# duj12/ASR-2Pass

Hardware: AMD Instinct MI355X
Metric: audio-sec/sec (xRT) Paraformer-large offline, 30s utts (higher is better)
Workload: dtype f32 (operands staged as 2 fp16 planes = 22-23 significant bits, 3 products per block on the FP16 matrix cores, fp32 accumulate; error vs fp64 = the fp32 MFMA chain's)

## Files before the change

asr-2pass_amd/csrc/attention_x3.hip:

```cpp
#include "kernels.h"
#include "launch_common.h"
#include "split_common.h"

#include <math.h>

namespace pfhip {
namespace {

using f32x16 = __attribute__((ext_vector_type(16))) float;

#ifndef PFHIP_ATT_ABLATE
#define PFHIP_ATT_ABLATE 0
#endif
constexpr bool kAbNoFsmn = PFHIP_ATT_ABLATE == 1, kAbNoBar = PFHIP_ATT_ABLATE == 2 || PFHIP_ATT_ABLATE == 6,
               kAbNoSoftmax = PFHIP_ATT_ABLATE == 3 || PFHIP_ATT_ABLATE == 6, kAbOneV = PFHIP_ATT_ABLATE == 4 || PFHIP_ATT_ABLATE == 6,
               kAbNoStage = PFHIP_ATT_ABLATE == 5 || PFHIP_ATT_ABLATE == 6;
constexpr int kHD = 128, kQW = 32, kNW = 8, kQB = kNW * kQW, kKT = 32;
constexpr int kKRow = 272;
constexpr int kKPlane = kKT * kKRow;
constexpr int kVRow = 72;
constexpr int kVPlane = kHD * kVRow;
constexpr int kBuf = 2 * kKPlane + 2 * kVPlane;
constexpr int kOS = kHD + 4;
constexpr int kLdsBytes = kNW * kQW * kOS * 4;
static_assert(kLdsBytes >= 2 * kBuf, "K/V buffers must fit");


__global__ __launch_bounds__(512, 1) void attention_x3_kernel(
    const float* __restrict__ Q, int ldq, const float* __restrict__ K, int ldk, const float* __restrict__ V, int ldv,
    float* __restrict__ O, int ldo, const int* __restrict__ q_off, const int* __restrict__ q_len,
    const int* __restrict__ kv_off, const int* __restrict__ kv_len, float scale, const float* __restrict__ fsmn_w,
    float* mem, int ldmem, int mem_accumulate, unsigned char* __restrict__ Ph, unsigned char* __restrict__ Pl, int rows_p) {
  extern __shared__ __attribute__((aligned(16))) unsigned char lds[];

  const int b = blockIdx.y, head = blockIdx.x;
  const int Lq = q_len[b];
  const int q0 = blockIdx.z * kQB;
  if (q0 >= Lq) return;
  const int Lk = kv_len[b];
  const size_t qbase = (size_t)q_off[b], kbase = (size_t)kv_off[b];
  const int tid = threadIdx.x, lane = tid & 63, wave = tid >> 6;
  const int r = lane & 31, h = lane >> 5;

  if (fsmn_w && !kAbNoFsmn) {
    constexpr int kTaps = 11, kStrip = 16;
    const int cg = tid & 31, strip = tid >> 5;
    const int c = head * kHD + 4 * cg, t0 = q0 + strip * kStrip;
    if (t0 < Lk) {
      float wk[4][kTaps];
#pragma unroll
      for (int ch = 0; ch < 4; ++ch)
#pragma unroll
        for (int j = 0; j < kTaps; ++j) wk[ch][j] = fsmn_w[(size_t)(c + ch) * kTaps + j];
      float4 rows[kStrip + kTaps - 1];
#pragma unroll
      for (int j = 0; j < kStrip + kTaps - 1; ++j) {
        const int t = t0 - 5 + j;
        rows[j] = (t < 0 || t >= Lk) ? make_float4(0.f, 0.f, 0.f, 0.f) : *reinterpret_cast<const float4*>(V + (kbase + t) * ldv + c);
      }
#pragma unroll
      for (int s0 = 0; s0 < kStrip; s0 += 8) {
        float4 xo[8];
#pragma unroll
        for (int s = 0; s < 8; ++s) {
          const int t = t0 + s0 + s;
          xo[s] = (mem_accumulate && t < Lk) ? *reinterpret_cast<const float4*>(mem + (kbase + t) * ldmem + c)
                                             : make_float4(0.f, 0.f, 0.f, 0.f);
        }
#pragma unroll
        for (int s1 = 0; s1 < 8; ++s1) {
          const int s = s0 + s1, t = t0 + s;
          if (t < Lk) {
            float4 o = rows[s + 5];
            float4 a = make_float4(0.f, 0.f, 0.f, 0.f);
#pragma unroll
            for (int j = 0; j < kTaps; ++j) {
              a.x += wk[0][j] * rows[s + j].x;
              a.y += wk[1][j] * rows[s + j].y;
              a.z += wk[2][j] * rows[s + j].z;
              a.w += wk[3][j] * rows[s + j].w;
            }
            o.x += a.x; o.y += a.y; o.z += a.z; o.w += a.w;
            if (mem_accumulate) { o.x += xo[s1].x; o.y += xo[s1].y; o.z += xo[s1].z; o.w += xo[s1].w; }
            *reinterpret_cast<float4*>(mem + (kbase + t) * ldmem + c) = o;
          }
        }
      }
    }
  }

  half8 qf[8][2];
  {
    int qrow = q0 + wave * kQW + r;
    if (qrow >= Lq) qrow = Lq - 1;
    const float* qp = Q + (qbase + qrow) * ldq + head * kHD + 8 * h;
    const float qs = scale * 1.44269504088896340736f;
#pragma unroll
    for (int s = 0; s < 8; ++s) {
      const float4 a = *reinterpret_cast<const float4*>(qp + 16 * s);
      const float4 c = *reinterpret_cast<const float4*>(qp + 16 * s + 4);
      const float v[8] = {a.x * qs, a.y * qs, a.z * qs, a.w * qs, c.x * qs, c.y * qs, c.z * qs, c.w * qs};
      split8(v, qf[s][0], qf[s][1]);
    }
  }

  const int kkey = tid >> 4, kc = tid & 15;
  const float* Kh = K + kbase * ldk + head * kHD + 4 * kc;
  const int vd2 = tid & 63, vkg = tid >> 6;
  const float* Vh = V + kbase * ldv + head * kHD + 2 * vd2;
  float4 rk0, rk1;
  float2 rv0, rv1, rv2, rv3;
  auto load_tile = [&](int kt) {
    int key = kt * kKT + kkey;
    key = key < Lk ? key : Lk - 1;
    const float* kp = Kh + (size_t)key * ldk;
    rk0 = *reinterpret_cast<const float4*>(kp);
    rk1 = *reinterpret_cast<const float4*>(kp + 64);
    const int k0 = kt * kKT + 4 * vkg;
    const int last = Lk - 1;
    rv0 = *reinterpret_cast<const float2*>(Vh + (size_t)min(k0, last) * ldv);
    rv1 = *reinterpret_cast<const float2*>(Vh + (size_t)min(k0 + 1, last) * ldv);
    rv2 = *reinterpret_cast<const float2*>(Vh + (size_t)min(k0 + 2, last) * ldv);
    rv3 = *reinterpret_cast<const float2*>(Vh + (size_t)min(k0 + 3, last) * ldv);
  };
  auto store4 = [&](float a, float c, float e, float g, unsigned char* base, int plane_bytes) {
    const unsigned h0 = hi_pair(a, c), h1 = hi_pair(e, g);
    *reinterpret_cast<uint2*>(base) = make_uint2(h0, h1);
    *reinterpret_cast<uint2*>(base + plane_bytes) = make_uint2(lo_pair(sub_lo(a, h0), sub_hi(c, h0)), lo_pair(sub_lo(e, h1), sub_hi(g, h1)));
  };
  auto store_tile = [&](int buf) {
    unsigned char* kb = lds + buf * kBuf + kkey * kKRow + 8 * kc;
    store4(rk0.x, rk0.y, rk0.z, rk0.w, kb, kKPlane);
    store4(rk1.x, rk1.y, rk1.z, rk1.w, kb + 128, kKPlane);
    unsigned char* vb = lds + buf * kBuf + 2 * kKPlane + (2 * vd2) * kVRow + 8 * vkg;
    store4(rv0.x, rv1.x, rv2.x, rv3.x, vb, kVPlane);
    store4(rv0.y, rv1.y, rv2.y, rv3.y, vb + kVRow, kVPlane);
  };

  f32x16 oacc0, oacc1, oacc2, oacc3;
#pragma unroll
  for (int e = 0; e < 16; ++e) { oacc0[e] = 0.f; oacc1[e] = 0.f; oacc2[e] = 0.f; oacc3[e] = 0.f; }
  float m_run = -1e30f, l_run = 0.f;

  const int nkt = (Lk + kKT - 1) / kKT;
  load_tile(0);
  store_tile(0);
  load_tile(nkt > 1 ? 1 : 0);
  __syncthreads();

  for (int kt = 0; kt < nkt; ++kt) {
    const int cur = kt & 1;
    const unsigned char* kb = lds + cur * kBuf + r * kKRow + 16 * h;
    const unsigned char* vb = lds + cur * kBuf + 2 * kKPlane + r * kVRow + 8 * h;

    f32x16 sacc;
#pragma unroll
    for (int e = 0; e < 16; ++e) sacc[e] = 0.f;
    unsigned char* const kst = lds + (cur ^ 1) * kBuf + kkey * kKRow + 8 * kc;
    unsigned char* const vst = lds + (cur ^ 1) * kBuf + 2 * kKPlane + (2 * vd2) * kVRow + 8 * vkg;
    unsigned th0, th1;
    float t0, t1, t2, t3;
#define PFHIP_SB __builtin_amdgcn_sched_barrier(0)
#define PFHIP_KF(dst, p, s_) dst = __builtin_bit_cast(half8, *reinterpret_cast<const uint4*>(kb + (p) * kKPlane + 32 * (s_)))
#define PFHIP_MM(a_, b_) sacc = __builtin_amdgcn_mfma_f32_32x32x16_f16(a_, b_, sacc, 0, 0, 0)
#define PFHIP_HI(a_, c_, e_, g_, dst)                                                                     \
  if (!kAbNoStage) { th0 = hi_pair(a_, c_); th1 = hi_pair(e_, g_); *reinterpret_cast<uint2*>(dst) = make_uint2(th0, th1);  \
    t0 = sub_lo(a_, th0); t1 = sub_hi(c_, th0); t2 = sub_lo(e_, th1); t3 = sub_hi(g_, th1); }
#define PFHIP_LO(dst) if (!kAbNoStage) { *reinterpret_cast<uint2*>(dst) = make_uint2(lo_pair(t0, t1), lo_pair(t2, t3)); }
    half8 k0, k1, n0, n1;
    PFHIP_KF(k0, 0, 0); PFHIP_KF(k1, 1, 0);
    PFHIP_SB;
    PFHIP_MM(k1, qf[0][0]); PFHIP_SB;
    PFHIP_KF(n0, 0, 1); PFHIP_KF(n1, 1, 1); PFHIP_SB;
    PFHIP_MM(k0, qf[0][1]); PFHIP_SB;
    PFHIP_HI(rk0.x, rk0.y, rk0.z, rk0.w, kst) PFHIP_SB;
    PFHIP_MM(k0, qf[0][0]); PFHIP_SB;
    PFHIP_MM(n1, qf[1][0]); PFHIP_SB;
    PFHIP_KF(k0, 0, 2); PFHIP_KF(k1, 1, 2); PFHIP_SB;
    PFHIP_MM(n0, qf[1][1]); PFHIP_SB;
    PFHIP_LO(kst + kKPlane) PFHIP_SB;
    PFHIP_MM(n0, qf[1][0]); PFHIP_SB;
    PFHIP_MM(k1, qf[2][0]); PFHIP_SB;
    PFHIP_KF(n0, 0, 3); PFHIP_KF(n1, 1, 3); PFHIP_SB;
    PFHIP_MM(k0, qf[2][1]); PFHIP_SB;
    PFHIP_HI(rk1.x, rk1.y, rk1.z, rk1.w, kst + 128) PFHIP_SB;
    PFHIP_MM(k0, qf[2][0]); PFHIP_SB;
    PFHIP_MM(n1, qf[3][0]); PFHIP_SB;
    PFHIP_KF(k0, 0, 4); PFHIP_KF(k1, 1, 4); PFHIP_SB;
    PFHIP_MM(n0, qf[3][1]); PFHIP_SB;
    PFHIP_LO(kst + 128 + kKPlane) PFHIP_SB;
    PFHIP_MM(n0, qf[3][0]); PFHIP_SB;
    PFHIP_MM(k1, qf[4][0]); PFHIP_SB;
    PFHIP_KF(n0, 0, 5); PFHIP_KF(n1, 1, 5); PFHIP_SB;
    PFHIP_MM(k0, qf[4][1]); PFHIP_SB;
    PFHIP_HI(rv0.x, rv1.x, rv2.x, rv3.x, vst) PFHIP_SB;
    PFHIP_MM(k0, qf[4][0]); PFHIP_SB;
    PFHIP_MM(n1, qf[5][0]); PFHIP_SB;
    PFHIP_KF(k0, 0, 6); PFHIP_KF(k1, 1, 6); PFHIP_SB;
    PFHIP_MM(n0, qf[5][1]); PFHIP_SB;
    PFHIP_LO(vst + kVPlane) PFHIP_SB;
    PFHIP_MM(n0, qf[5][0]); PFHIP_SB;
    PFHIP_MM(k1, qf[6][0]); PFHIP_SB;
    PFHIP_KF(n0, 0, 7); PFHIP_KF(n1, 1, 7); PFHIP_SB;
    PFHIP_MM(k0, qf[6][1]); PFHIP_SB;
    PFHIP_HI(rv0.y, rv1.y, rv2.y, rv3.y, vst + kVRow) PFHIP_SB;
    PFHIP_MM(k0, qf[6][0]); PFHIP_SB;
    PFHIP_MM(n1, qf[7][0]); PFHIP_SB;
    PFHIP_MM(n0, qf[7][1]); PFHIP_SB;
    PFHIP_LO(vst + kVRow + kVPlane) PFHIP_SB;
    PFHIP_MM(n0, qf[7][0]); PFHIP_SB;
#undef PFHIP_LO
#undef PFHIP_HI
#undef PFHIP_MM
#undef PFHIP_KF
#undef PFHIP_SB
    __builtin_amdgcn_sched_barrier(0);
    if (!kAbNoStage) load_tile(kt + 2 < nkt ? kt + 2 : nkt - 1);
    __builtin_amdgcn_sched_barrier(0);

    float tmax = -INFINITY;
    if (kAbNoSoftmax) {
      tmax = m_run;
    } else if ((kt + 1) * kKT <= Lk) {
#pragma unroll
      for (int e = 0; e < 16; ++e) tmax = fmaxf(tmax, sacc[e]);
    } else {
      const int key0 = kt * kKT + 4 * h;
#pragma unroll
      for (int e = 0; e < 16; ++e) {
        const int key = key0 + (e & 3) + 8 * (e >> 2);
        const float sv = (key < Lk) ? sacc[e] : -INFINITY;
        sacc[e] = sv;
        tmax = fmaxf(tmax, sv);
      }
    }
    tmax = fmaxf(tmax, __shfl_xor(tmax, 32));
    if (__any(tmax > m_run + 10.0f)) {
      const float m_new = fmaxf(m_run, tmax);
      const float alpha = __builtin_amdgcn_exp2f(m_run - m_new);
      l_run *= alpha;
      m_run = m_new;
#pragma unroll
      for (int e = 0; e < 16; ++e) { oacc0[e] *= alpha; oacc1[e] *= alpha; oacc2[e] *= alpha; oacc3[e] *= alpha; }
    }
    float psum = 0.f;
#pragma unroll
    for (int e = 0; e < 16; ++e) {
      const float pv = kAbNoSoftmax ? sacc[e] : __builtin_amdgcn_exp2f(sacc[e] - m_run);
      sacc[e] = pv;
      psum += pv;
    }
    psum += __shfl_xor(psum, 32);
    l_run += psum;

#pragma unroll
    for (int t = 0; t < 2; ++t) {
      const float pv[8] = {sacc[8 * t + 0], sacc[8 * t + 1], sacc[8 * t + 2], sacc[8 * t + 3],
                           sacc[8 * t + 4], sacc[8 * t + 5], sacc[8 * t + 6], sacc[8 * t + 7]};
      half8 p0, p1;
      split8(pv, p0, p1);
#define PFHIP_PV(OACC, dt)                                                                                        \
      {                                                                                                           \
        const unsigned char* vp = kAbOneV ? vb : vb + (dt) * 32 * kVRow + 32 * t;                                 \
        half8 v0, v1;                                                                                             \
        {                                                                                                         \
          const uint2 lo = *reinterpret_cast<const uint2*>(vp), hi = *reinterpret_cast<const uint2*>(vp + 16);    \
          v0 = __builtin_bit_cast(half8, make_uint4(lo.x, lo.y, hi.x, hi.y));                                     \
        }                                                                                                         \
        {                                                                                                         \
          const uint2 lo = *reinterpret_cast<const uint2*>(vp + kVPlane), hi = *reinterpret_cast<const uint2*>(vp + kVPlane + 16); \
          v1 = __builtin_bit_cast(half8, make_uint4(lo.x, lo.y, hi.x, hi.y));                                     \
        }                                                                                                         \
        OACC = __builtin_amdgcn_mfma_f32_32x32x16_f16(v1, p0, OACC, 0, 0, 0);                                     \
        OACC = __builtin_amdgcn_mfma_f32_32x32x16_f16(v0, p1, OACC, 0, 0, 0);                                     \
        OACC = __builtin_amdgcn_mfma_f32_32x32x16_f16(v0, p0, OACC, 0, 0, 0);                                     \
      }
      PFHIP_PV(oacc0, 0) PFHIP_PV(oacc1, 1) PFHIP_PV(oacc2, 2) PFHIP_PV(oacc3, 3)
#undef PFHIP_PV
    }
    if (!kAbNoBar) __syncthreads();
  }

  const float inv_l = 1.0f / l_run;
  float* os = reinterpret_cast<float*>(lds) + wave * (kQW * kOS);
#define PFHIP_O_STORE(OACC, dt)                                                          \
  _Pragma("unroll") for (int g = 0; g < 4; ++g) {                                        \
    float4 o4;                                                                           \
    o4.x = OACC[4 * g + 0] * inv_l; o4.y = OACC[4 * g + 1] * inv_l;                      \
    o4.z = OACC[4 * g + 2] * inv_l; o4.w = OACC[4 * g + 3] * inv_l;                      \
    *reinterpret_cast<float4*>(os + r * kOS + (dt) * 32 + 8 * g + 4 * h) = o4;           \
  }
  PFHIP_O_STORE(oacc0, 0) PFHIP_O_STORE(oacc1, 1) PFHIP_O_STORE(oacc2, 2) PFHIP_O_STORE(oacc3, 3)
#undef PFHIP_O_STORE
  __syncthreads();
  if (Ph) {
    const int pc = h, qrow = q0 + wave * kQW + r;
    const size_t grow = qbase + (size_t)qrow;
    if (qrow < Lq) {
#pragma unroll
      for (int ks = 0; ks < kHD / 16; ++ks) {
        const float4 a = *reinterpret_cast<const float4*>(os + r * kOS + 16 * ks + 8 * pc);
        const float4 c = *reinterpret_cast<const float4*>(os + r * kOS + 16 * ks + 8 * pc + 4);
        const float v[8] = {a.x, a.y, a.z, a.w, c.x, c.y, c.z, c.w};
        half8 p0, p1;
        split8(v, p0, p1);
        const size_t off = ((size_t)(head * (kHD / 16) + ks) * rows_p + grow) * 32 + (size_t)((pc ^ (int)((grow >> 3) & 1)) << 4);
        *reinterpret_cast<uint4*>(Ph + off) = __builtin_bit_cast(uint4, p0);
        *reinterpret_cast<uint4*>(Pl + off) = __builtin_bit_cast(uint4, p1);
      }
    }
  } else {
    constexpr int C4 = kHD / 4, RW = 64 / C4;
#pragma unroll
    for (int pass = 0; pass < kQW / RW; ++pass) {
      const int row = pass * RW + lane / C4, cc = lane % C4;
      const int qrow = q0 + wave * kQW + row;
      if (qrow < Lq) {
        const float4 o4 = *reinterpret_cast<const float4*>(os + row * kOS + 4 * cc);
        *reinterpret_cast<float4*>(O + (qbase + qrow) * ldo + head * kHD + 4 * cc) = o4;
      }
    }
  }
}

}

void launch_attention_x3(const float* Q, int ldq, const float* K, int ldk, const float* V, int ldv, float* O, int ldo,
                         const int* q_off, const int* q_len, const int* kv_off, const int* kv_len, int B, int H, int max_q_len,
                         float scale, hipStream_t s, const float* fsmn_w, float* mem, int ldmem, bool mem_accumulate, void* planes_hi,
                         void* planes_lo, int plane_rows) {
  if (B <= 0 || max_q_len <= 0) return;
  const dim3 grid(H, B, (max_q_len + kQB - 1) / kQB);
  launch_with_lds<attention_x3_kernel>(grid, kLdsBytes, s, Q, ldq, K, ldk, V, ldv, O, ldo, q_off, q_len, kv_off,
                     kv_len, scale, fsmn_w, mem, ldmem, mem_accumulate ? 1 : 0, static_cast<unsigned char*>(planes_hi),
                     static_cast<unsigned char*>(planes_lo), plane_rows);
}

}
```

Baseline: 40820.

## Software-pipeline attention so QK^T of next tile overlaps softmax and PV of current

Restructures the flash-attention loop into a three-buffer LDS ring, computing the S=QK^T MFMAs for tile kt+1 while doing exp/split softmax of tile kt and interleaving the PV MFMAs with the fp16 hi/lo staging of tile kt+2. K and V global loads are split and issued three tiles ahead. The aim is to hide softmax VALU work and LDS staging behind matrix-core issue. The cost is extra LDS use, two live score accumulators (more VGPR pressure) and a more intricate hand-scheduled sequence with a prologue and epilogue.

```diff
diff --git a/asr-2pass_amd/csrc/attention_x3.hip b/asr-2pass_amd/csrc/attention_x3.hip
--- a/asr-2pass_amd/csrc/attention_x3.hip
+++ b/asr-2pass_amd/csrc/attention_x3.hip
@@ -23,7 +23,7 @@
 constexpr int kBuf = 2 * kKPlane + 2 * kVPlane;
 constexpr int kOS = kHD + 4;
 constexpr int kLdsBytes = kNW * kQW * kOS * 4;
-static_assert(kLdsBytes >= 2 * kBuf, "K/V buffers must fit");
+static_assert(kLdsBytes >= 3 * kBuf, "K/V buffers must fit");
 
 
 __global__ __launch_bounds__(512, 1) void attention_x3_kernel(
@@ -110,12 +110,14 @@
   const float* Vh = V + kbase * ldv + head * kHD + 2 * vd2;
   float4 rk0, rk1;
   float2 rv0, rv1, rv2, rv3;
-  auto load_tile = [&](int kt) {
+  auto load_k = [&](int kt) {
     int key = kt * kKT + kkey;
     key = key < Lk ? key : Lk - 1;
     const float* kp = Kh + (size_t)key * ldk;
     rk0 = *reinterpret_cast<const float4*>(kp);
     rk1 = *reinterpret_cast<const float4*>(kp + 64);
+  };
+  auto load_v = [&](int kt) {
     const int k0 = kt * kKT + 4 * vkg;
     const int last = Lk - 1;
     rv0 = *reinterpret_cast<const float2*>(Vh + (size_t)min(k0, last) * ldv);
@@ -128,14 +130,10 @@
     *reinterpret_cast<uint2*>(base) = make_uint2(h0, h1);
     *reinterpret_cast<uint2*>(base + plane_bytes) = make_uint2(lo_pair(sub_lo(a, h0), sub_hi(c, h0)), lo_pair(sub_lo(e, h1), sub_hi(g, h1)));
   };
-  auto store_tile = [&](int buf) {
-    unsigned char* kb = lds + buf * kBuf + kkey * kKRow + 8 * kc;
-    store4(rk0.x, rk0.y, rk0.z, rk0.w, kb, kKPlane);
-    store4(rk1.x, rk1.y, rk1.z, rk1.w, kb + 128, kKPlane);
-    unsigned char* vb = lds + buf * kBuf + 2 * kKPlane + (2 * vd2) * kVRow + 8 * vkg;
-    store4(rv0.x, rv1.x, rv2.x, rv3.x, vb, kVPlane);
-    store4(rv0.y, rv1.y, rv2.y, rv3.y, vb + kVRow, kVPlane);
-  };
+  unsigned char* const kstage = lds + kkey * kKRow + 8 * kc;
+  unsigned char* const vstage = lds + 2 * kKPlane + (2 * vd2) * kVRow + 8 * vkg;
+  const unsigned char* const kfrag = lds + r * kKRow + 16 * h;
+  const unsigned char* const vfrag = lds + 2 * kKPlane + r * kVRow + 8 * h;
 
   f32x16 oacc0, oacc1, oacc2, oacc3;
 #pragma unroll
@@ -143,81 +141,253 @@
   float m_run = -1e30f, l_run = 0.f;
 
   const int nkt = (Lk + kKT - 1) / kKT;
-  load_tile(0);
-  store_tile(0);
-  load_tile(nkt > 1 ? 1 : 0);
+  const int last_kt = max(nkt - 1, 0);
+  load_k(0);
+  load_v(0);
+  store4(rk0.x, rk0.y, rk0.z, rk0.w, kstage, kKPlane);
+  store4(rk1.x, rk1.y, rk1.z, rk1.w, kstage + 128, kKPlane);
+  store4(rv0.x, rv1.x, rv2.x, rv3.x, vstage, kVPlane);
+  store4(rv0.y, rv1.y, rv2.y, rv3.y, vstage + kVRow, kVPlane);
+  load_k(min(1, last_kt));
+  load_v(min(1, last_kt));
   __syncthreads();
 
-  for (int kt = 0; kt < nkt; ++kt) {
-    const int cur = kt & 1;
-    const unsigned char* kb = lds + cur * kBuf + r * kKRow + 16 * h;
-    const unsigned char* vb = lds + cur * kBuf + 2 * kKPlane + r * kVRow + 8 * h;
-
-    f32x16 sacc;
-#pragma unroll
-    for (int e = 0; e < 16; ++e) sacc[e] = 0.f;
-    unsigned char* const kst = lds + (cur ^ 1) * kBuf + kkey * kKRow + 8 * kc;
-    unsigned char* const vst = lds + (cur ^ 1) * kBuf + 2 * kKPlane + (2 * vd2) * kVRow + 8 * vkg;
-    unsigned th0, th1;
-    float t0, t1, t2, t3;
 #define PFHIP_SB __builtin_amdgcn_sched_barrier(0)
 #define PFHIP_KF(dst, p, s_) dst = __builtin_bit_cast(half8, *reinterpret_cast<const uint4*>(kb + (p) * kKPlane + 32 * (s_)))
-#define PFHIP_MM(a_, b_) sacc = __builtin_amdgcn_mfma_f32_32x32x16_f16(a_, b_, sacc, 0, 0, 0)
+#define PFHIP_MM(S_, a_, b_) S_ = __builtin_amdgcn_mfma_f32_32x32x16_f16(a_, b_, S_, 0, 0, 0)
 #define PFHIP_HI(a_, c_, e_, g_, dst)                                                                     \
   if (!kAbNoStage) { th0 = hi_pair(a_, c_); th1 = hi_pair(e_, g_); *reinterpret_cast<uint2*>(dst) = make_uint2(th0, th1);  \
     t0 = sub_lo(a_, th0); t1 = sub_hi(c_, th0); t2 = sub_lo(e_, th1); t3 = sub_hi(g_, th1); }
 #define PFHIP_LO(dst) if (!kAbNoStage) { *reinterpret_cast<uint2*>(dst) = make_uint2(lo_pair(t0, t1), lo_pair(t2, t3)); }
+  unsigned th0, th1;
+  float t0, t1, t2, t3;
+
+  f32x16 sA, sB;
+  {
+#pragma unroll
+    for (int e = 0; e < 16; ++e) sA[e] = 0.f;
+    const unsigned char* kb = kfrag;
+    unsigned char* const kst = kstage + kBuf;
+    unsigned char* const vst = vstage + kBuf;
     half8 k0, k1, n0, n1;
     PFHIP_KF(k0, 0, 0); PFHIP_KF(k1, 1, 0);
     PFHIP_SB;
-    PFHIP_MM(k1, qf[0][0]); PFHIP_SB;
+    PFHIP_MM(sA, k1, qf[0][0]); PFHIP_SB;
     PFHIP_KF(n0, 0, 1); PFHIP_KF(n1, 1, 1); PFHIP_SB;
-    PFHIP_MM(k0, qf[0][1]); PFHIP_SB;
+    PFHIP_MM(sA, k0, qf[0][1]); PFHIP_SB;
     PFHIP_HI(rk0.x, rk0.y, rk0.z, rk0.w, kst) PFHIP_SB;
-    PFHIP_MM(k0, qf[0][0]); PFHIP_SB;
-    PFHIP_MM(n1, qf[1][0]); PFHIP_SB;
+    PFHIP_MM(sA, k0, qf[0][0]); PFHIP_SB;
+    PFHIP_MM(sA, n1, qf[1][0]); PFHIP_SB;
     PFHIP_KF(k0, 0, 2); PFHIP_KF(k1, 1, 2); PFHIP_SB;
-    PFHIP_MM(n0, qf[1][1]); PFHIP_SB;
+    PFHIP_MM(sA, n0, qf[1][1]); PFHIP_SB;
     PFHIP_LO(kst + kKPlane) PFHIP_SB;
-    PFHIP_MM(n0, qf[1][0]); PFHIP_SB;
-    PFHIP_MM(k1, qf[2][0]); PFHIP_SB;
+    PFHIP_MM(sA, n0, qf[1][0]); PFHIP_SB;
+    PFHIP_MM(sA, k1, qf[2][0]); PFHIP_SB;
     PFHIP_KF(n0, 0, 3); PFHIP_KF(n1, 1, 3); PFHIP_SB;
-    PFHIP_MM(k0, qf[2][1]); PFHIP_SB;
+    PFHIP_MM(sA, k0, qf[2][1]); PFHIP_SB;
     PFHIP_HI(rk1.x, rk1.y, rk1.z, rk1.w, kst + 128) PFHIP_SB;
-    PFHIP_MM(k0, qf[2][0]); PFHIP_SB;
-    PFHIP_MM(n1, qf[3][0]); PFHIP_SB;
+    PFHIP_MM(sA, k0, qf[2][0]); PFHIP_SB;
+    PFHIP_MM(sA, n1, qf[3][0]); PFHIP_SB;
     PFHIP_KF(k0, 0, 4); PFHIP_KF(k1, 1, 4); PFHIP_SB;
-    PFHIP_MM(n0, qf[3][1]); PFHIP_SB;
+    PFHIP_MM(sA, n0, qf[3][1]); PFHIP_SB;
     PFHIP_LO(kst + 128 + kKPlane) PFHIP_SB;
-    PFHIP_MM(n0, qf[3][0]); PFHIP_SB;
-    PFHIP_MM(k1, qf[4][0]); PFHIP_SB;
+    PFHIP_MM(sA, n0, qf[3][0]); PFHIP_SB;
+    PFHIP_MM(sA, k1, qf[4][0]); PFHIP_SB;
     PFHIP_KF(n0, 0, 5); PFHIP_KF(n1, 1, 5); PFHIP_SB;
-    PFHIP_MM(k0, qf[4][1]); PFHIP_SB;
+    PFHIP_MM(sA, k0, qf[4][1]); PFHIP_SB;
     PFHIP_HI(rv0.x, rv1.x, rv2.x, rv3.x, vst) PFHIP_SB;
-    PFHIP_MM(k0, qf[4][0]); PFHIP_SB;
-    PFHIP_MM(n1, qf[5][0]); PFHIP_SB;
+    PFHIP_MM(sA, k0, qf[4][0]); PFHIP_SB;
+    PFHIP_MM(sA, n1, qf[5][0]); PFHIP_SB;
     PFHIP_KF(k0, 0, 6); PFHIP_KF(k1, 1, 6); PFHIP_SB;
-    PFHIP_MM(n0, qf[5][1]); PFHIP_SB;
+    PFHIP_MM(sA, n0, qf[5][1]); PFHIP_SB;
     PFHIP_LO(vst + kVPlane) PFHIP_SB;
-    PFHIP_MM(n0, qf[5][0]); PFHIP_SB;
-    PFHIP_MM(k1, qf[6][0]); PFHIP_SB;
+    PFHIP_MM(sA, n0, qf[5][0]); PFHIP_SB;
+    PFHIP_MM(sA, k1, qf[6][0]); PFHIP_SB;
     PFHIP_KF(n0, 0, 7); PFHIP_KF(n1, 1, 7); PFHIP_SB;
-    PFHIP_MM(k0, qf[6][1]); PFHIP_SB;
+    PFHIP_MM(sA, k0, qf[6][1]); PFHIP_SB;
     PFHIP_HI(rv0.y, rv1.y, rv2.y, rv3.y, vst + kVRow) PFHIP_SB;
-    PFHIP_MM(k0, qf[6][0]); PFHIP_SB;
-    PFHIP_MM(n1, qf[7][0]); PFHIP_SB;
-    PFHIP_MM(n0, qf[7][1]); PFHIP_SB;
+    PFHIP_MM(sA, k0, qf[6][0]); PFHIP_SB;
+    PFHIP_MM(sA, n1, qf[7][0]); PFHIP_SB;
+    PFHIP_MM(sA, n0, qf[7][1]); PFHIP_SB;
     PFHIP_LO(vst + kVRow + kVPlane) PFHIP_SB;
-    PFHIP_MM(n0, qf[7][0]); PFHIP_SB;
+    PFHIP_MM(sA, n0, qf[7][0]); PFHIP_SB;
+    if (!kAbNoStage) { load_k(min(2, last_kt)); load_v(min(2, last_kt)); }
+    PFHIP_SB;
+    __syncthreads();
+  }
+
+  auto rescale = [&](float tmax) __attribute__((always_inline)) {
+    if (__any(tmax > m_run + 10.0f)) {
+      const float m_new = fmaxf(m_run, tmax);
+      const float alpha = __builtin_amdgcn_exp2f(m_run - m_new);
+      l_run *= alpha;
+      m_run = m_new;
+#pragma unroll
+      for (int e = 0; e < 16; ++e) { oacc0[e] *= alpha; oacc1[e] *= alpha; oacc2[e] *= alpha; oacc3[e] *= alpha; }
+    }
+  };
+
+  int kt = 0;
+  int o_cur = 0, o_nxt = kBuf, o_nn = 2 * kBuf;
+  auto tile_step = [&](f32x16 scur) __attribute__((always_inline)) -> f32x16 {
+    f32x16 snext;
+    const unsigned char* kb = kfrag + o_nxt;
+    const unsigned char* vb = vfrag + o_cur;
+    unsigned char* const kst = kstage + o_nn;
+    unsigned char* const vst = vstage + o_nn;
+#pragma unroll
+    for (int e = 0; e < 16; ++e) snext[e] = 0.f;
+
+    half8 k0, k1, n0, n1;
+    float tmax = -INFINITY;
+    PFHIP_KF(k0, 0, 0); PFHIP_KF(k1, 1, 0);
+    PFHIP_SB;
+    PFHIP_MM(snext, k1, qf[0][0]); PFHIP_SB;
+    PFHIP_KF(n0, 0, 1); PFHIP_KF(n1, 1, 1); PFHIP_SB;
+    if (!kAbNoSoftmax) {
+#pragma unroll
+      for (int e = 0; e < 8; ++e) tmax = fmaxf(tmax, scur[e]);
+    }
+    PFHIP_SB;
+    PFHIP_MM(snext, k0, qf[0][1]); PFHIP_SB;
+    if (!kAbNoSoftmax) {
+#pragma unroll
+      for (int e = 8; e < 16; ++e) tmax = fmaxf(tmax, scur[e]);
+    }
+    PFHIP_SB;
+    PFHIP_MM(snext, k0, qf[0][0]); PFHIP_SB;
+    if (kAbNoSoftmax) tmax = m_run; else tmax = fmaxf(tmax, __shfl_xor(tmax, 32));
+    rescale(tmax);
+    float psum = 0.f;
+    half8 pa0, pa1, pb0, pb1;
+#define PFHIP_EXP4(e0)                                                                                     \
+    _Pragma("unroll") for (int e = (e0); e < (e0) + 4; ++e) {                                               \
+      const float pv = kAbNoSoftmax ? scur[e] : __builtin_amdgcn_exp2f(scur[e] - m_run);                   \
+      scur[e] = pv;                                                                                        \
+      psum += pv;                                                                                          \
+    }
+#define PFHIP_SPLIT(t, p0, p1)                                                                             \
+    {                                                                                                      \
+      const float pv[8] = {scur[8 * (t) + 0], scur[8 * (t) + 1], scur[8 * (t) + 2], scur[8 * (t) + 3],     \
+                           scur[8 * (t) + 4], scur[8 * (t) + 5], scur[8 * (t) + 6], scur[8 * (t) + 7]};    \
+      split8(pv, p0, p1);                                                                                  \
+    }
+    PFHIP_SB;
+    PFHIP_MM(snext, n1, qf[1][0]); PFHIP_SB;
+    PFHIP_KF(k0, 0, 2); PFHIP_KF(k1, 1, 2); PFHIP_SB;
+    PFHIP_MM(snext, n0, qf[1][1]); PFHIP_SB;
+    PFHIP_EXP4(0) PFHIP_SB;
+    PFHIP_MM(snext, n0, qf[1][0]); PFHIP_SB;
+    PFHIP_MM(snext, k1, qf[2][0]); PFHIP_SB;
+    PFHIP_KF(n0, 0, 3); PFHIP_KF(n1, 1, 3); PFHIP_SB;
+    PFHIP_MM(snext, k0, qf[2][1]); PFHIP_SB;
+    PFHIP_EXP4(4) PFHIP_SB;
+    PFHIP_MM(snext, k0, qf[2][0]); PFHIP_SB;
+    PFHIP_MM(snext, n1, qf[3][0]); PFHIP_SB;
+    PFHIP_KF(k0, 0, 4); PFHIP_KF(k1, 1, 4); PFHIP_SB;
+    PFHIP_MM(snext, n0, qf[3][1]); PFHIP_SB;
+    PFHIP_SPLIT(0, pa0, pa1) PFHIP_SB;
+    PFHIP_MM(snext, n0, qf[3][0]); PFHIP_SB;
+    PFHIP_MM(snext, k1, qf[4][0]); PFHIP_SB;
+    PFHIP_KF(n0, 0, 5); PFHIP_KF(n1, 1, 5); PFHIP_SB;
+    PFHIP_MM(snext, k0, qf[4][1]); PFHIP_SB;
+    PFHIP_EXP4(8) PFHIP_SB;
+    PFHIP_MM(snext, k0, qf[4][0]); PFHIP_SB;
+    PFHIP_MM(snext, n1, qf[5][0]); PFHIP_SB;
+    PFHIP_KF(k0, 0, 6); PFHIP_KF(k1, 1, 6); PFHIP_SB;
+    PFHIP_MM(snext, n0, qf[5][1]); PFHIP_SB;
+    PFHIP_EXP4(12) PFHIP_SB;
+    PFHIP_MM(snext, n0, qf[5][0]); PFHIP_SB;
+    PFHIP_MM(snext, k1, qf[6][0]); PFHIP_SB;
+    PFHIP_KF(n0, 0, 7); PFHIP_KF(n1, 1, 7); PFHIP_SB;
+    PFHIP_MM(snext, k0, qf[6][1]); PFHIP_SB;
+    PFHIP_SPLIT(1, pb0, pb1) PFHIP_SB;
+    PFHIP_MM(snext, k0, qf[6][0]); PFHIP_SB;
+    PFHIP_MM(snext, n1, qf[7][0]); PFHIP_SB;
+    PFHIP_MM(snext, n0, qf[7][1]); PFHIP_SB;
+    const float psum_other = __shfl_xor(psum, 32);
+    PFHIP_SB;
+    PFHIP_MM(snext, n0, qf[7][0]); PFHIP_SB;
+#undef PFHIP_SPLIT
+#undef PFHIP_EXP4
+
+#define PFHIP_VF(d0, d1, t, dt)                                                                                      \
+    {                                                                                                                \
+      const unsigned char* vp = kAbOneV ? vb : vb + (dt) * 32 * kVRow + 32 * (t);                                    \
+      const uint2 a0 = *reinterpret_cast<const uint2*>(vp), a1 = *reinterpret_cast<const uint2*>(vp + 16);           \
+      const uint2 c0 = *reinterpret_cast<const uint2*>(vp + kVPlane), c1 = *reinterpret_cast<const uint2*>(vp + kVPlane + 16); \
+      d0 = __builtin_bit_cast(half8, make_uint4(a0.x, a0.y, a1.x, a1.y));                                            \
+      d1 = __builtin_bit_cast(half8, make_uint4(c0.x, c0.y, c1.x, c1.y));                                            \
+    }
+    half8 v0, v1, w0, w1;
+    PFHIP_VF(v0, v1, 0, 0) PFHIP_SB;
+    PFHIP_MM(oacc0, v1, pa0); PFHIP_SB;
+    psum += psum_other;
+    l_run += psum;
+    PFHIP_VF(w0, w1, 0, 1) PFHIP_SB;
+    PFHIP_MM(oacc0, v0, pa1); PFHIP_SB;
+    PFHIP_HI(rk0.x, rk0.y, rk0.z, rk0.w, kst) PFHIP_SB;
+    PFHIP_MM(oacc0, v0, pa0); PFHIP_SB;
+    PFHIP_MM(oacc1, w1, pa0); PFHIP_SB;
+    PFHIP_VF(v0, v1, 0, 2) PFHIP_SB;
+    PFHIP_MM(oacc1, w0, pa1); PFHIP_SB;
+    PFHIP_LO(kst + kKPlane) PFHIP_SB;
+    PFHIP_MM(oacc1, w0, pa0); PFHIP_SB;
+    PFHIP_MM(oacc2, v1, pa0); PFHIP_SB;
+    PFHIP_VF(w0, w1, 0, 3) PFHIP_SB;
+    PFHIP_MM(oacc2, v0, pa1); PFHIP_SB;
+    PFHIP_HI(rk1.x, rk1.y, rk1.z, rk1.w, kst + 128) PFHIP_SB;
+    PFHIP_MM(oacc2, v0, pa0); PFHIP_SB;
+    PFHIP_MM(oacc3, w1, pa0); PFHIP_SB;
+    PFHIP_VF(v0, v1, 1, 0) PFHIP_SB;
+    PFHIP_MM(oacc3, w0, pa1); PFHIP_SB;
+    PFHIP_LO(kst + 128 + kKPlane) PFHIP_SB;
+    PFHIP_MM(oacc3, w0, pa0); PFHIP_SB;
+    if (!kAbNoStage) load_k(min(kt + 3, last_kt));
+    PFHIP_SB;
+    PFHIP_MM(oacc0, v1, pb0); PFHIP_SB;
+    PFHIP_VF(w0, w1, 1, 1) PFHIP_SB;
+    PFHIP_MM(oacc0, v0, pb1); PFHIP_SB;
+    PFHIP_HI(rv0.x, rv1.x, rv2.x, rv3.x, vst) PFHIP_SB;
+    PFHIP_MM(oacc0, v0, pb0); PFHIP_SB;
+    PFHIP_MM(oacc1, w1, pb0); PFHIP_SB;
+    PFHIP_VF(v0, v1, 1, 2) PFHIP_SB;
+    PFHIP_MM(oacc1, w0, pb1); PFHIP_SB;
+    PFHIP_LO(vst + kVPlane) PFHIP_SB;
+    PFHIP_MM(oacc1, w0, pb0); PFHIP_SB;
+    PFHIP_MM(oacc2, v1, pb0); PFHIP_SB;
+    PFHIP_VF(w0, w1, 1, 3) PFHIP_SB;
+    PFHIP_MM(oacc2, v0, pb1); PFHIP_SB;
+    PFHIP_HI(rv0.y, rv1.y, rv2.y, rv3.y, vst + kVRow) PFHIP_SB;
+    PFHIP_MM(oacc2, v0, pb0); PFHIP_SB;
+    PFHIP_MM(oacc3, w1, pb0); PFHIP_SB;
+    PFHIP_MM(oacc3, w0, pb1); PFHIP_SB;
+    PFHIP_LO(vst + kVRow + kVPlane) PFHIP_SB;
+    PFHIP_MM(oacc3, w0, pb0); PFHIP_SB;
+    if (!kAbNoStage) load_v(min(kt + 3, last_kt));
+    PFHIP_SB;
+#undef PFHIP_VF
+    if (!kAbNoBar) __syncthreads();
+    ++kt;
+    const int o = o_cur;
+    o_cur = o_nxt; o_nxt = o_nn; o_nn = o;
+    return snext;
+  };
+  f32x16 sacc;
+  for (;;) {
+    if (kt >= last_kt) { sacc = sA; break; }
+    sB = tile_step(sA);
+    if (kt >= last_kt) { sacc = sB; break; }
+    sA = tile_step(sB);
+  }
 #undef PFHIP_LO
 #undef PFHIP_HI
 #undef PFHIP_MM
 #undef PFHIP_KF
 #undef PFHIP_SB
-    __builtin_amdgcn_sched_barrier(0);
-    if (!kAbNoStage) load_tile(kt + 2 < nkt ? kt + 2 : nkt - 1);
-    __builtin_amdgcn_sched_barrier(0);
-
+
+  {
+    const unsigned char* vb = vfrag + o_cur;
     float tmax = -INFINITY;
     if (kAbNoSoftmax) {
       tmax = m_run;
@@ -235,14 +405,7 @@
       }
     }
     tmax = fmaxf(tmax, __shfl_xor(tmax, 32));
-    if (__any(tmax > m_run + 10.0f)) {
-      const float m_new = fmaxf(m_run, tmax);
-      const float alpha = __builtin_amdgcn_exp2f(m_run - m_new);
-      l_run *= alpha;
-      m_run = m_new;
-#pragma unroll
-      for (int e = 0; e < 16; ++e) { oacc0[e] *= alpha; oacc1[e] *= alpha; oacc2[e] *= alpha; oacc3[e] *= alpha; }
-    }
+    rescale(tmax);
     float psum = 0.f;
 #pragma unroll
     for (int e = 0; e < 16; ++e) {
@@ -252,7 +415,6 @@
     }
     psum += __shfl_xor(psum, 32);
     l_run += psum;
-
 #pragma unroll
     for (int t = 0; t < 2; ++t) {
       const float pv[8] = {sacc[8 * t + 0], sacc[8 * t + 1], sacc[8 * t + 2], sacc[8 * t + 3],
@@ -278,7 +440,9 @@
       PFHIP_PV(oacc0, 0) PFHIP_PV(oacc1, 1) PFHIP_PV(oacc2, 2) PFHIP_PV(oacc3, 3)
 #undef PFHIP_PV
     }
-    if (!kAbNoBar) __syncthreads();
+    asm volatile("" ::"v"(rk0.x), "v"(rk0.y), "v"(rk0.z), "v"(rk0.w), "v"(rk1.x), "v"(rk1.y), "v"(rk1.z), "v"(rk1.w), "v"(rv0.x), "v"(rv0.y),
+                 "v"(rv1.x), "v"(rv1.y), "v"(rv2.x), "v"(rv2.y), "v"(rv3.x), "v"(rv3.y));
+    __syncthreads();
   }
 
   const float inv_l = 1.0f / l_run;
```

Result: no change. 41020 (median of 6 runs) (+0.5%).
